# ZJU-DAILY/HC-SpMM

Hardware: AMD Instinct MI355X
Metric: GNN-aggregation SpMM edges*dim/s (A*X, fp32) (higher is better)
Workload: dtype f32

## Files before the change

hc-spmm_amd/csrc/capi.hip:

```cpp
#include <hip/hip_runtime.h>
#include <stdint.h>
#include <stdlib.h>

#include "fingerprint.h"
#include "graph_build.h"
#include "hcspmm.h"
#include "spmm_kernels.h"

namespace {
thread_local int g_last_hip_error = 0;

int fail_hip(hipError_t e) {
  g_last_hip_error = (int)e;
  return HCSPMM_EHIP;
}

inline bool aligned(const void* p, size_t a) { return (reinterpret_cast<uintptr_t>(p) & (a - 1)) == 0; }

constexpr int kDtypeF8 = HCSPMM_DTYPE_BF16 + 1;

inline int elem_bytes(int dtype) { return dtype == HCSPMM_DTYPE_F32 ? 4 : dtype == kDtypeF8 ? 1 : 2; }

int pick_vec(int dtype, int D, int64_t ldx, int64_t ldz, const void* X, const void* Z, const void* ws) {
  if (dtype == HCSPMM_DTYPE_F32) return D >= 4 ? 4 : D >= 2 ? 2 : 1;
// ... 233 lines not shown
  p.off_sched = ph->off_tasks;
  p.n_tasks = ph->n_tasks;
  p.n_tiny = ph->n_tiny;
  p.off_slice_table = ph->off_slice_table;
  p.off_slice_tasks = ph->off_slice_tasks;
  p.n_slices = ph->n_slices;
  p.slice_xcd_tasks = ph->slice_xcd_tasks;
  p.off_dense_index = ph->off_dense_index;
  p.off_dense_pack = ph->off_dense_pack;
  p.n_dense = ph->n_dense;
  p.off_dense_compact = ph->off_dense_compact;
  p.n_dense_compact = ph->n_dense_compact;
  p.off_dense_compact2 = ph->off_dense_compact2;
  p.n_dense_compact2 = ph->n_dense_compact2;
  p.off_fixups = ph->off_fixups;
  p.n_split_rows = ph->n_split_rows;
  wide_choice(ph, D, dtype, &p.n_wide, &p.panel_cols);
  return HCSPMM_OK;
}

inline void use_schedule(hcspmm::PlanArgs& p, const hcspmm_plan_header* ph) {
  if (ph->off_task_sched != 0) p.off_sched = ph->off_task_sched;
  if (ph->off_slice_sched != 0) p.off_slice_tasks = ph->off_slice_sched;
}

inline void set_operands(hcspmm::PlanArgs& p, const void* X, void* Z, int64_t ldx, int64_t ldz) {
  p.X = X;
  p.Z = Z;
  p.ldx = (size_t)ldx;
  p.ldz = (size_t)ldz;
}

inline hcspmm::WindowArgs window_args(const GraphIn& g, const hcspmm::PlanArgs& p) {
  return hcspmm::WindowArgs{p.X, p.Z, g.rowptr, g.col, g.blockPartition, g.edgeToColumn, g.edgeToRow, g.hybrid_type, p.ldx, p.ldz,
                            p.N, p.D};
}

template <class A>
using Launcher = hipError_t (*)(const A&, int, hipStream_t);
template <class A>
hipError_t launch_typed(int dtype, Launcher<A> f32, Launcher<A> f16, Launcher<A> bf16, const A& a, int vec, hipStream_t stream) {
  return (dtype == HCSPMM_DTYPE_F32 ? f32 : dtype == HCSPMM_DTYPE_F16 ? f16 : bf16)(a, vec, stream);
}

int forward_impl(const void* X, int64_t x_rows, int64_t ldx, void* Z, int64_t ldz, int dtype, const GraphIn& g, int D,
                 void* workspace, size_t workspace_bytes, void* stream_v, const FusedOperands* fused, const float* values = nullptr,
// ... 670 lines not shown
```

hc-spmm_amd/csrc/plan_host.cpp:

```cpp
#include <algorithm>
#include <atomic>
#include <chrono>
#include <condition_variable>
#include <cstdint>
#include <cstdio>
#include <cstdlib>
#include <cstring>
#include <mutex>
#include <thread>
#include <vector>

#include "fingerprint.h"
#include "hcspmm.h"
#include "host_util.h"

namespace {

constexpr int kSliceAuto = 0, kSliceOn = 1, kSliceOff = -1;
constexpr int32_t kSliceAutoThreshold = 256;
constexpr int64_t kSliceAutoMinColumns = 65536;
constexpr int64_t kSliceAutoAlwaysColumns = 250000;
constexpr int64_t kSliceAutoMinEntries = 3000000;
constexpr int kSliceSample = 4;
constexpr int64_t kScheduleMaxColumns = (256ll << 20) / 128;
constexpr int kSlicePad = 64;

struct Resolved {
  int32_t split_threshold, segment_len, fuse_in_launch;
  int32_t slice_mode, slice_threshold, n_slices, panel_cols;
  int32_t schedule;
};

int env_int(const char* name, int dflt) {
  const char* e = std::getenv(name);
  return e && *e ? std::atoi(e) : dflt;
}

Resolved resolve(const hcspmm_plan_params* p) {
  Resolved r{512, 256, 0, kSliceAuto, kSliceAutoThreshold, 8, 0, -1};
  if (p) {
    if (p->split_threshold > 0) r.split_threshold = p->split_threshold;
    if (p->segment_len > 0) r.segment_len = p->segment_len;
    r.fuse_in_launch = p->fuse_in_launch < 0 ? -1 : (p->fuse_in_launch > 2 ? 2 : p->fuse_in_launch);
  }
  if (r.segment_len > r.split_threshold) r.segment_len = r.split_threshold;
  int thr = p ? p->slice_threshold : 0, ns = p ? p->n_slices : 0;
  if (thr == 0) thr = env_int("HCSPMM_SLICE_THRESHOLD", 0);
  if (ns == 0) ns = env_int("HCSPMM_SLICES", 0);
  if (thr > 0) { r.slice_mode = kSliceOn; r.slice_threshold = thr; }
  else if (thr < 0) r.slice_mode = kSliceOff;
  if (ns > 0) r.n_slices = std::min(64, (ns + 7) / 8 * 8);
  r.schedule = env_int("HCSPMM_TASK_SCHEDULE", -1);
  if (p && p->panel_cols != 0) r.panel_cols = p->panel_cols < 0 ? -1 : std::min(1 << 20, (p->panel_cols + 15) / 16 * 16);
  return r;
}

inline int64_t pieces_bound(int64_t d, const Resolved& rp) {
  return std::min<int64_t>(d, rp.n_slices - 1 + (d + rp.segment_len - 1) / rp.segment_len);
}

inline void slice_cuts(const int32_t* col, int32_t e0, int64_t d, const int32_t* bounds, int S, int32_t* cuts) {
  const int32_t* first = col + e0;
  int64_t lo = 0;
  cuts[0] = 0;
  for (int s = 0; s < S; ++s) {
    const int64_t hi = (s == S - 1) ? d : std::lower_bound(first + lo, first + d, bounds[s]) - first;
    cuts[s + 1] = (int32_t)hi;
    lo = hi;
  }
}

template <typename F>
inline void for_each_piece(const int32_t* cuts, int32_t e0, int S, int32_t seg, F fn) {
  for (int s = 0; s < S; ++s)
    for (int64_t b = cuts[s]; b < cuts[s + 1]; b += seg) fn(s, (int32_t)(e0 + b), (int32_t)std::min<int64_t>(seg, cuts[s + 1] - b));
}

inline int64_t align4(int64_t x) { return (x + 3) & ~int64_t(3); }

struct Layout {
  int64_t n_tasks = 0, n_tiny = 0, n_dense = 0, n_compact = 0, n_compact2 = 0, n_split_rows = 0, n_partials = 0;
  int64_t dense_pack_words = 0;
  int64_t nnz_sparse = 0, nnz_dense = 0, dense_k_sum = 0;
  int32_t max_dense_k = 0;
  int64_t n_sparse_windows = 0;
  int64_t n_slice_tasks = 0, n_sliced_rows = 0, nnz_sliced = 0;
  int64_t off_tasks = 0, off_dense_index = 0, off_dense_pack = 0, off_compact2 = 0, off_compact = 0, off_fixups = 0,
          off_sparse_windows = 0, off_slice_table = 0, off_slice_tasks = 0, off_task_sched = 0, off_slice_sched = 0, total = 0;
};

class PassPool {
 public:
  explicit PassPool(int T) : T_(T) {
    for (int t = 1; t < T_; ++t) th_.emplace_back([this, t] { work(t); });
  }
  ~PassPool() {
    fn_ = nullptr;
    post();
    for (auto& x : th_) x.join();
  }
  int size() const { return T_; }
  template <typename F> void run(F& fn) {
    fn_ = [](void* f, int t) { (*static_cast<F*>(f))(t); };
    arg_ = &fn;
    done_.store(0, std::memory_order_relaxed);
    post();
    fn(0);
    for (int spin = 0; done_.load(std::memory_order_acquire) != T_ - 1; ++spin)
      if (spin > 256) std::this_thread::yield();
  }

// ... 104 lines not shown
    L.nnz_sparse += p.nnz_sparse; L.nnz_dense += p.nnz_dense; L.dense_k_sum += p.dense_k_sum;
    L.n_sparse_windows += p.n_sparse_windows;
    L.n_slice_tasks += p.n_slice_tasks; L.n_sliced_rows += p.n_sliced_rows; L.nnz_sliced += p.nnz_sliced;
    L.max_dense_k = std::max(L.max_dense_k, p.max_dense_k);
  }
  if (slicing) L.n_slice_tasks += (int64_t)kSlicePad * rp.n_slices;
  L.off_tasks = HCSPMM_PLAN_HEADER_WORDS;
  L.off_dense_index = align4(L.off_tasks + 4 * L.n_tasks);
  L.off_dense_pack = align4(L.off_dense_index + 4 * L.n_dense);
  L.off_compact2 = (L.off_dense_pack + L.dense_pack_words + 63) & ~int64_t(63);
  L.off_compact = L.off_compact2 + HCSPMM_COMPACT2_WORDS * L.n_compact2;
  L.off_fixups = align4(L.off_compact + HCSPMM_COMPACT_WORDS * L.n_compact);
  L.off_sparse_windows = align4(L.off_fixups + 4 * L.n_split_rows);
  L.off_slice_table = align4(L.off_sparse_windows + L.n_sparse_windows);
  L.off_slice_tasks = slicing ? align4(L.off_slice_table + rp.n_slices + 1) : L.off_slice_table;
  L.total = align4(L.off_slice_tasks + 4 * (slicing ? L.n_slice_tasks : 0));
  if (rp.schedule) {
    L.off_task_sched = L.total;
    L.total += 4 * (L.n_tasks - L.n_tiny);
    if (slicing) {
      L.off_slice_sched = L.total;
      L.total += 4 * L.n_slice_tasks;
    }
  }
  if (L.total > INT32_MAX) return HCSPMM_ERANGE;
  *out = L;
  return HCSPMM_OK;
}

void sort_by_length(const int32_t* src, int32_t* dst, int64_t n, int32_t max_len, int T) {
  if (n <= 0) return;
  if (n < 65536) T = 1;
  int32_t longest = 0;
  {
    std::vector<int32_t> part((size_t)T, 0);
    parallel_for(T, [&](int t) {
      int32_t m = 0;
      for (int64_t i = n * t / T; i < n * (t + 1) / T; ++i) m = std::max(m, src[4 * i + 2]);
      part[(size_t)t] = m;
    });
    for (int t = 0; t < T; ++t) longest = std::max(longest, part[(size_t)t]);
  }
  longest = std::min(longest, max_len);
  const size_t nb = (size_t)longest + 1;
  if (nb * (size_t)T > ((size_t)1 << 24)) T = 1;
  std::vector<std::vector<int64_t>> at((size_t)T);
  parallel_for(T, [&](int t) {
    std::vector<int64_t> h(nb, 0);
    for (int64_t i = n * t / T; i < n * (t + 1) / T; ++i) h[(size_t)std::min(std::max(src[4 * i + 2], 0), longest)]++;
    at[(size_t)t].swap(h);
// ... 75 lines not shown
}

extern "C" int hcspmm_plan_build(const int32_t* rowptr, const int32_t* col, int64_t N, int64_t E, int64_t M,
                                 const int32_t* bp, const int32_t* e2c, const int32_t* ht,
                                 const hcspmm_plan_params* params, int32_t* plan, int64_t words) {
  if (!rowptr || !plan || N < 0 || E < 0) return HCSPMM_EINVAL;
  if (N > 0 && (!bp || !ht)) return HCSPMM_EINVAL;
  if (E > 0 && (!col || !e2c)) return HCSPMM_EINVAL;
  if (N > INT32_MAX - 16 || E > INT32_MAX) return HCSPMM_ERANGE;
  if (M <= 0) M = N;
  if (M > INT32_MAX) return HCSPMM_ERANGE;
  PoolScope scope(plan_threads((N + HCSPMM_BLK_H - 1) / HCSPMM_BLK_H));
  static const bool dbg = std::getenv("HCSPMM_PLAN_DEBUG") != nullptr;
  auto now = [] { return std::chrono::duration<double, std::milli>(std::chrono::steady_clock::now().time_since_epoch()).count(); };
  double tp[8] = {now(), 0, 0, 0, 0, 0, 0, 0};
  uint64_t fingerprint = 0;
  {
    const int frc = fingerprint_and_check(rowptr, col, N, E, M, &fingerprint);
    if (frc != HCSPMM_OK) return frc;
  }
  tp[1] = now();
  Resolved rp = resolve(params);
  rp.schedule = rp.schedule < 0 ? (M <= kScheduleMaxColumns) : (rp.schedule != 0);
  Layout L;
  int rc = HCSPMM_OK;
  bool slicing = rp.slice_mode == kSliceOn;
  if (rp.slice_mode != kSliceOff) {
    rc = compute_layout(rowptr, N, bp, ht, rp, true, &L);
    if (rc != HCSPMM_OK) return rc;
    if (rp.slice_mode == kSliceAuto)
      slicing = M >= kSliceAutoMinColumns && L.nnz_sliced * 20 >= L.nnz_sparse && L.nnz_sliced > 0 &&
                (M >= kSliceAutoAlwaysColumns || L.nnz_sparse >= kSliceAutoMinEntries);
    if (L.n_sliced_rows == 0) slicing = false;
  }
  if (!slicing) {
    rc = compute_layout(rowptr, N, bp, ht, rp, false, &L);
    if (rc != HCSPMM_OK) return rc;
  }
  if (words < L.total) return HCSPMM_EINVAL;
  const int64_t W = (N + HCSPMM_BLK_H - 1) / HCSPMM_BLK_H;
  const int S = slicing ? rp.n_slices : 0;
  tp[2] = now();

  const int T = plan_threads(W);
  std::vector<int64_t> cut((size_t)T + 1);
  for (int t = 0; t <= T; ++t) cut[(size_t)t] = W * t / T;
// ... 204 lines not shown
         [&](int sl, int32_t row, int32_t first, int32_t len, int32_t slot_id) {
           const int64_t q = sp[(size_t)sl * (size_t)n_cls + (size_t)length_class(len)]++;
           sout[4 * q + 0] = row;
           sout[4 * q + 1] = first;
           sout[4 * q + 2] = len;
           sout[4 * q + 3] = slot_id;
         });
  });

  if (rp.schedule) {
    const int64_t n_nt = L.n_tasks - L.n_tiny;
    sort_by_length(out, plan + L.off_task_sched, n_nt, rp.split_threshold, T);
    if (slicing) {
      int32_t* ssched = plan + L.off_slice_sched;
      std::atomic<int> next_list{0};
      parallel_for(T, [&](int) {
        for (int sl; (sl = next_list.fetch_add(1, std::memory_order_relaxed)) < S;) {
          const int64_t lo = table[(size_t)sl], real = slice_real[(size_t)sl];
          sort_by_length(sout + 4 * lo, ssched + 4 * lo, real, rp.split_threshold, 1);
          std::memcpy(ssched + 4 * (lo + real), sout + 4 * (lo + real), 16 * (size_t)(table[(size_t)sl + 1] - lo - real));
        }
      });
      std::memset(ssched + 4 * table[(size_t)S], 0, 16 * (size_t)(L.n_slice_tasks - table[(size_t)S]));
    }
  }

  tp[5] = now();
  std::stable_sort(dense.begin(), dense.end(), [](const DenseRef& a, const DenseRef& b) { return a.K > b.K; });
  int32_t* dindex = plan + L.off_dense_index;
  int32_t* dpack = plan + L.off_dense_pack;
  const int64_t n_reg = L.n_dense - L.n_compact - L.n_compact2, n_c2 = L.n_compact2;
  std::vector<int64_t> pack_at((size_t)n_reg + 1, 0);
  for (int64_t i = 0; i < n_reg; ++i) pack_at[(size_t)i + 1] = pack_at[(size_t)i] + dense[(size_t)i].K + (dense[(size_t)i].K / 4) * 2;
  std::vector<int64_t> uniq_part((size_t)T, 0);
  std::vector<int> bad((size_t)T, 0);
  parallel_for(T, [&](int t) {
    int64_t uniq_total = 0;
    for (int64_t i = L.n_dense * t / T; i < L.n_dense * (t + 1) / T; ++i) {
      const int64_t w = dense[(size_t)i].w;
      const int32_t K = dense[(size_t)i].K, K4 = K / 4;
      const int64_t r0 = w * HCSPMM_BLK_H, r1 = std::min<int64_t>(r0 + HCSPMM_BLK_H, N);
      const int kind = i < n_reg ? 0 : (i < n_reg + n_c2 ? 2 : 1);
      if (kind != (K <= HCSPMM_COMPACT_K ? 1 : (K <= HCSPMM_COMPACT2_K ? 2 : 0))) { bad[(size_t)t] = 1; return; }
      const int32_t kmax = kind == 1 ? HCSPMM_COMPACT_K : (kind == 2 ? HCSPMM_COMPACT2_K : K);
      const int64_t off = kind == 1 ? HCSPMM_COMPACT_WORDS * (i - n_reg - n_c2)
                                    : (kind == 2 ? HCSPMM_COMPACT2_WORDS * (i - n_reg) : pack_at[(size_t)i]);
// ... 54 lines not shown
  h.n_tiny = (int32_t)n_tiny;
  h.n_dense_compact = (int32_t)L.n_compact;
  h.off_dense_compact = (int32_t)L.off_compact;
  h.n_dense_compact2 = (int32_t)L.n_compact2;
  h.off_dense_compact2 = (int32_t)L.off_compact2;
  h.num_columns = (int32_t)M;
  h.n_sparse_windows = (int32_t)L.n_sparse_windows;
  h.off_sparse_windows = (int32_t)L.off_sparse_windows;
  h.fingerprint_lo = (uint32_t)(fingerprint & 0xffffffffull);
  h.fingerprint_hi = (uint32_t)(fingerprint >> 32);
  h.dense_k_sum = (int32_t)std::min<int64_t>(L.dense_k_sum, INT32_MAX);
  h.flags = rp.fuse_in_launch < 0 ? HCSPMM_PLAN_FUSE_NEVER : (rp.fuse_in_launch >= 2 ? HCSPMM_PLAN_FUSE_ROWS : (rp.fuse_in_launch == 1 ? HCSPMM_PLAN_FUSE_IN_LAUNCH : 0));
  h.n_slices = S;
  h.slice_threshold = slicing ? rp.slice_threshold : 0;
  h.off_slice_table = (int32_t)L.off_slice_table;
  h.off_slice_tasks = (int32_t)L.off_slice_tasks;
  h.n_slice_tasks = slicing ? (int32_t)table[(size_t)S] : 0;
  h.slice_xcd_tasks = (int32_t)slice_xcd_tasks;
  h.nnz_sliced = slicing ? (int32_t)L.nnz_sliced : 0;
  h.n_sliced_rows = slicing ? (int32_t)L.n_sliced_rows : 0;
  h.panel_cols = rp.panel_cols;
  h.off_task_sched = (int32_t)L.off_task_sched;
  h.off_slice_sched = (int32_t)L.off_slice_sched;
  static_assert(sizeof(hcspmm_plan_header) == HCSPMM_PLAN_HEADER_WORDS * 4, "header size");
  std::memcpy(plan, &h, sizeof(h));
  if (dbg) {
    tp[6] = now();
    std::fprintf(stderr, "plan_build: T=%d: fingerprint + range check %.2f | layout %.2f | clear + slice boundaries %.2f | task pass 1 (count) %.2f | "
                         "task pass 2 (write) %.2f | dense packs %.2f | total %.2f ms\n",
                 T, tp[1] - tp[0], tp[2] - tp[1], tp[3] - tp[2], tp[4] - tp[3], tp[5] - tp[4], tp[6] - tp[5], tp[6] - tp[0]);
  }
  return HCSPMM_OK;
}

extern "C" int hcspmm_plan_check(const hcspmm_plan_header* h, int64_t N, int64_t E, int64_t words_available) {
  if (!h) return HCSPMM_EINVAL;
  if (h->magic != HCSPMM_PLAN_MAGIC || h->version != HCSPMM_PLAN_VERSION) return HCSPMM_EPLAN;
  if (h->num_nodes != N || h->num_edges != E) return HCSPMM_EPLAN;
  if (h->num_windows != (N + HCSPMM_BLK_H - 1) / HCSPMM_BLK_H) return HCSPMM_EPLAN;
  if (h->num_columns < 0 || (h->num_columns == 0 && N > 0)) return HCSPMM_EPLAN;
  if (h->n_tasks < 0 || h->n_dense < 0 || h->n_split_rows < 0 || h->n_partials < 0) return HCSPMM_EPLAN;
  if (h->n_tiny < 0 || h->n_tiny > h->n_tasks) return HCSPMM_EPLAN;
  if (h->n_dense_compact < 0 || h->n_dense_compact2 < 0 ||
      (int64_t)h->n_dense_compact + h->n_dense_compact2 > h->n_dense)
    return HCSPMM_EPLAN;
  if (h->n_sparse_windows < 0 || (int64_t)h->n_sparse_windows + h->n_dense != h->num_windows) return HCSPMM_EPLAN;
// ... 13 lines not shown
  if (h->off_sparse_windows < h->off_fixups + 4 * (int64_t)h->n_split_rows || (h->off_sparse_windows & 3)) return HCSPMM_EPLAN;
  if (h->total_words < h->off_sparse_windows + (int64_t)h->n_sparse_windows) return HCSPMM_EPLAN;
  if (h->n_slices < 0 || h->n_slices > 64 || (h->n_slices & 7) || h->n_slice_tasks < 0 || h->slice_xcd_tasks < 0) return HCSPMM_EPLAN;
  if (h->n_slices > 0) {
    if (h->slice_threshold <= 0 || (h->n_slice_tasks % 64) || (h->slice_xcd_tasks % 64) || h->slice_xcd_tasks > h->n_slice_tasks)
      return HCSPMM_EPLAN;
    if (h->off_slice_table < h->off_sparse_windows + (int64_t)h->n_sparse_windows || (h->off_slice_table & 3)) return HCSPMM_EPLAN;
    if (h->off_slice_tasks < h->off_slice_table + (int64_t)h->n_slices + 1 || (h->off_slice_tasks & 3)) return HCSPMM_EPLAN;
    if (h->total_words < h->off_slice_tasks + 4 * (int64_t)h->n_slice_tasks) return HCSPMM_EPLAN;
    if (h->nnz_sliced < 0 || h->nnz_sliced > h->nnz_sparse) return HCSPMM_EPLAN;
  } else if (h->n_slice_tasks != 0 || h->slice_xcd_tasks != 0) {
    return HCSPMM_EPLAN;
  }
  const int64_t lists_end = h->n_slices > 0 ? h->off_slice_tasks + 4 * (int64_t)h->n_slice_tasks
                                            : h->off_sparse_windows + (int64_t)h->n_sparse_windows;
  const int64_t n_nt = (int64_t)h->n_tasks - h->n_tiny;
  if (h->off_task_sched != 0 &&
      (h->off_task_sched < lists_end || (h->off_task_sched & 3) || h->total_words < h->off_task_sched + 4 * n_nt))
    return HCSPMM_EPLAN;
  if (h->off_slice_sched != 0 &&
      (h->n_slices == 0 || h->off_task_sched == 0 || h->off_slice_sched < h->off_task_sched + 4 * n_nt || (h->off_slice_sched & 3) ||
       h->total_words < h->off_slice_sched + 4 * (int64_t)h->n_slice_tasks))
    return HCSPMM_EPLAN;
  if (words_available > 0 && h->total_words > words_available) return HCSPMM_EPLAN;
  if ((int64_t)h->nnz_sparse + h->nnz_dense != E) return HCSPMM_EPLAN;
  return HCSPMM_OK;
}

extern "C" size_t hcspmm_workspace_bytes(const hcspmm_plan_header* h, int D) {
  if (!h || D <= 0) return 0;
  return (size_t)h->n_partials * (size_t)D * sizeof(float);
}
```

hc-spmm_amd/csrc/spmm_impl.h:

```cpp
#pragma once
#include <hip/hip_runtime.h>
#include <stdint.h>
#include <stdlib.h>

#include "hcspmm.h"
#include "spmm_kernels.h"
#include "plan_layout.h"

namespace hcspmm {

struct F32 { typedef float T; typedef float Z; };
struct F16 { typedef unsigned short T; typedef unsigned short Z; };
struct BF16 { typedef unsigned short T; typedef unsigned short Z; };
struct F8 { typedef unsigned char T; typedef float Z; };

typedef float f32x4 __attribute__((ext_vector_type(4)));
typedef unsigned int u32x4 __attribute__((ext_vector_type(4)));
typedef unsigned int u32x2 __attribute__((ext_vector_type(2)));

template <int VEC> struct AccT { typedef float type __attribute__((ext_vector_type(VEC))); };
template <> struct AccT<1> { typedef float type; };
__device__ __forceinline__ float aget(const float& v, int) { return v; }
__device__ __forceinline__ void aset(float& v, int, float x) { v = x; }
template <typename V> __device__ __forceinline__ float aget(const V& v, int i) { return v[i]; }
// ... 164 lines not shown
}

#ifndef HCSPMM_INDEX_VEC
#define HCSPMM_INDEX_VEC 4
#endif
#ifndef HCSPMM_INDEX_VEC_MIN
#define HCSPMM_INDEX_VEC_MIN 32
#endif

template <int IV>
__device__ __forceinline__ const int* index_source(const int* __restrict__ col, int e, int left, int nE,
                                                   typename IntV<IV>::type& v) {
  if (left <= 0) return nullptr;
  if constexpr (IV == 1) return col + e;
  else {
    if (e <= nE - IV) return col + e;
#pragma unroll
    for (int k = 0; k < IV; ++k)
      if (k < left) v[k] = col[e + k];
    return nullptr;
  }
}

template <typename E, int L, int VEC, bool WIDE, int UMAX, int IV>
__device__ __forceinline__ void sparse_task_body(const typename E::T* __restrict__ X, typename E::Z* __restrict__ dstZ,
                                                 float* __restrict__ dstP, const int* __restrict__ col, int nE, int e0, int n,
                                                 int nmax, size_t ldx, int c0, int cend, int lane) {
  typedef Lane<E, VEC> Ln;
  typedef typename Ln::acc_t acc_t;
  constexpr int U = (L < UMAX) ? L : UMAX;
  typedef typename IntV<IV>::type idx_t;
  typedef typename MemI32<IV>::type idx_mem_t;
  constexpr int STRIDE = WIDE ? 64 : L * IV;
  static_assert(IV == 1 || U % IV == 0, "a batch must start on a lane's first index");
  const int s = lane & (L - 1);
  const int pos = WIDE ? lane : s * IV;
  const int gbase = lane & ~(L - 1);

  for (int pbase = c0; pbase < cend; pbase += L * VEC) {
    const bool cok = pbase + s * VEC < cend;
    const int c = cok ? lane_col<VEC>(pbase + s * VEC, cend) : 0;
    const int csafe = c;
    acc_t acc = azero<VEC>();
    idx_t next = idx_t(-1);
    if (const int* p0 = index_source<IV>(col, e0 + pos, n - pos, nE, next)) next = *reinterpret_cast<const idx_mem_t*>(p0);
    for (int base = 0; base < nmax; base += STRIDE) {
      idx_t myidx = next;
      if constexpr (IV > 1) {
#pragma unroll
        for (int k = 1; k < IV; ++k) myidx[k] = (base + pos + k < n) ? myidx[k] : -1;
      }
      next = idx_t(-1);
      const int cnt = min(WIDE ? L : STRIDE, nmax - base);
      const int* pf = index_source<IV>(col, e0 + base + STRIDE + pos, n - (base + STRIDE + pos), nE, next);
      for (int j = 0; j < cnt;) {
        const int left = cnt - j;
        const int src = gbase + j / IV;
        if (left > U / 2) {
          gather_batch<E, VEC, U, IV>(X, ldx, csafe, cok, myidx, src, acc, pf, next);
          j += U;
        } else if (U >= 8 && left > U / 4) {
          gather_batch<E, VEC, (U >= 8 ? U / 2 : 1), IV>(X, ldx, csafe, cok, myidx, src, acc, pf, next);
          j += U / 2;
        } else if (U >= 4 && left > 1) {
          gather_batch<E, VEC, (U >= 8 ? U / 4 : 2), IV>(X, ldx, csafe, cok, myidx, src, acc, pf, next);
          j += (U >= 8 ? U / 4 : 2);
        } else {
          gather_batch<E, VEC, 1, IV>(X, ldx, csafe, cok, myidx, src, acc, pf, next);
          j += 1;
        }
        pf = nullptr;
      }
    }
    if (WIDE) {
#pragma unroll
      for (int off = L; off < 64; off <<= 1) {
#pragma unroll
        for (int q = 0; q < VEC; ++q) aset(acc, q, aget(acc, q) + __shfl_xor(aget(acc, q), off, 64));
      }
    }
    if (cok && (!WIDE || lane < L)) {
      if (dstZ != nullptr) Ln::store(dstZ + c, acc);
      else if (dstP != nullptr) Ln::store_partial(dstP + c, acc);
    }
  }
}

template <typename E, int L, int VEC, bool WIDE, int UMAX = HCSPMM_SPARSE_U, int IVREQ = 1>
__device__ __forceinline__ void sparse_task(const typename E::T* __restrict__ X, typename E::Z* __restrict__ dstZ,
                                            float* __restrict__ dstP, const int* __restrict__ col, int nE, int e0, int n,
                                            size_t ldx, int c0, int cend, int lane) {
  int nmax = n;
  if (!WIDE) {
#pragma unroll
    for (int off = L; off < 64; off <<= 1) nmax = max(nmax, __shfl_xor(nmax, off, 64));
  }
  nmax = __builtin_amdgcn_readfirstlane(nmax);
  constexpr int IV = (!WIDE && L == 8 && sizeof(typename E::T) == 4) ? IVREQ : 1;
  if constexpr (IV > 1) {
    if (nmax > HCSPMM_INDEX_VEC_MIN) {
      sparse_task_body<E, L, VEC, WIDE, UMAX, IV>(X, dstZ, dstP, col, nE, e0, n, nmax, ldx, c0, cend, lane);
      return;
    }
  }
  sparse_task_body<E, L, VEC, WIDE, UMAX, 1>(X, dstZ, dstP, col, nE, e0, n, nmax, ldx, c0, cend, lane);
}

template <typename E, int L, int VEC, int T>
__device__ __forceinline__ void tiny_tasks(const PlanArgs& a, int first, int c0, int cend, int lane) {
  typedef Lane<E, VEC> Ln;
  typedef typename E::T elem_t;
  const elem_t* X = reinterpret_cast<const elem_t*>(a.X);
  typename E::Z* Z = reinterpret_cast<typename E::Z*>(a.Z);
  constexpr int R = 64 / L;
  const int g = lane / L, s = lane & (L - 1);
  const int4* tasks = reinterpret_cast<const int4*>(a.plan + a.off_tasks);
  int4 d[T];
  bool any1 = false, any2 = false;
#pragma unroll
  for (int t = 0; t < T; ++t) {
    const int tid = first + t * R + g;
    d[t] = (tid < a.n_tasks) ? tasks[tid] : int4{0, -1, -1, -1};
  }
#pragma unroll
  for (int t = 0; t < T; ++t) {
    any1 |= d[t].y >= 0;
    any2 |= d[t].w >= 0;
  }
// ... 323 lines not shown
    const int p = (int)blockIdx.x / a.sparse_wgs_pp;
    const int b = (int)blockIdx.x - p * a.sparse_wgs_pp;
    const int c0 = p * a.panel_cols;
    const int cend = min(a.D, c0 + a.panel_cols);
    const int bf = b - a.slice_wgs;
    if (bf >= 0 && bf < a.wide_wgs) {
      const int tid = bf * kWaves + wave;
      if (tid >= a.n_wide) return;
      const int4 t = reinterpret_cast<const int4*>(a.plan + a.off_sched)[tid];
      typename E::Z* dz = (t.w < 0) ? Z + (size_t)t.x * a.ldz : nullptr;
      float* dp = (t.w < 0) ? nullptr : a.partial + (size_t)t.w * (size_t)a.D;
      sparse_task<E, L, VEC, true, UNROLL>(X, dz, dp, a.col, a.E, __builtin_amdgcn_readfirstlane(t.y),
                                           __builtin_amdgcn_readfirstlane(t.z), a.ldx, c0, cend, lane);
    } else if (bf >= sparse_wgs_pp_ordinary_end(a)) {
      if (bf >= a.free_wgs_pp) return;
      constexpr int R = 64 / L;
      const int first = a.n_tasks - a.n_tiny + ((bf - sparse_wgs_pp_ordinary_end(a)) * kWaves + wave) * (R * TinyT<L>::value);
      if (first >= a.n_tasks) return;
      tiny_tasks<E, L, VEC, TinyT<L>::value>(a, first, c0, cend, lane);
    } else {
      constexpr int R = 64 / L;
      const int g = lane / L;
      const int4* tp = nullptr;
      if (bf < 0) {
        cint_p tbl = (cint_p)(a.plan + a.off_slice_table);
        int j = ((b >> 3) * kWaves + wave) * R;
        for (int sl = b & 7; sl < a.n_slices; sl += 8) {
          const int lo = tbl[sl], cnt = tbl[sl + 1] - lo;
          if (j < cnt) {
            tp = reinterpret_cast<const int4*>(a.plan + a.off_slice_tasks) + lo + j + g;
            break;
          }
          j -= cnt;
        }
      } else {
        const int tid = a.n_wide + ((bf - a.wide_wgs) * kWaves + wave) * R + g;
        if (tid < a.n_tasks - a.n_tiny) tp = reinterpret_cast<const int4*>(a.plan + a.off_sched) + tid;
      }
      int e0 = 0, n = 0;
      typename E::Z* dz = nullptr;
      float* dp = nullptr;
      if (tp != nullptr) {
        const int4 t = *tp;
        if (t.x >= 0) {
          e0 = t.y;
          n = t.z;
          if (t.w < 0) dz = Z + (size_t)t.x * a.ldz;
          else dp = a.partial + (size_t)t.w * (size_t)a.D;
        }
      }
      sparse_task<E, L, VEC, false, UNROLL, HCSPMM_INDEX_VEC>(X, dz, dp, a.col, a.E, e0, n, a.ldx, c0, cend, lane);
    }
  } else {
    if constexpr (FUSED) {
      fused_dense_region(a, lane, wave);
      return;
    }
    constexpr int VM = DenseV<VEC>::mid;
    int unit = ((int)blockIdx.x - a.sparse_wgs) * kWaves + wave;
    if (unit >= a.n_dense * a.n_panels) return;
    const int n_reg = a.n_dense - a.n_dense_compact - a.n_dense_compact2;
    if (unit >= n_reg * a.n_panels) {
      unit -= n_reg * a.n_panels;
      if (unit < a.n_dense_compact2 * a.n_panels) {
        const int panel = unit / a.n_dense_compact2, ci = unit - panel * a.n_dense_compact2;
        const int* rec = a.plan + a.off_dense_compact2 + ci * HCSPMM_COMPACT2_WORDS;
        if (a.dense_vec == VEC) dense_compact_unit<E, VEC, 2>(X, Z, rec, panel, a.N, a.D, a.ldx, a.ldz, lane);
        else if (a.dense_vec == VM) dense_compact_unit<E, VM, 2>(X, Z, rec, panel, a.N, a.D, a.ldx, a.ldz, lane);
        else dense_compact_unit<E, 1, 2>(X, Z, rec, panel, a.N, a.D, a.ldx, a.ldz, lane);
        return;
      }
      unit -= a.n_dense_compact2 * a.n_panels;
      const int panel = unit / a.n_dense_compact, ci = unit - panel * a.n_dense_compact;
      const int* rec = a.plan + a.off_dense_compact + ci * HCSPMM_COMPACT_WORDS;
// ... 261 lines not shown
```

hc-spmm_amd/csrc/spmm_kernels.h:

```cpp
#pragma once
#include <hip/hip_runtime.h>
#include <stdint.h>

namespace hcspmm {

struct PlanArgs {
  const void* X;
  void* Z;
  float* partial;
  const int* col;
  const int* plan;
  size_t ldx, ldz;
  int off_tasks, n_tasks;
  int off_dense_index, off_dense_pack, n_dense;
  int off_dense_compact, n_dense_compact;
  int off_dense_compact2, n_dense_compact2;
  int off_fixups, n_split_rows;
  int N, D;
  int n_wide;
  int n_tiny;
  int panel_cols;
  int sparse_wgs_pp, dense_vec;
  int wide_wgs, sparse_wgs, n_panels;
  int tiny_wgs;
  int tiny_kernel_wgs;
  int off_slice_table, off_slice_tasks, n_slices, slice_xcd_tasks;
  int slice_wgs;
  int free_wgs_pp;
  int fused, H;
  int fused_dense_wgs;
  union {
    const float* W;
    const float* row_scale;
  };
  long long w_ldr, w_ldc;
  float* out;
  int E;
  int off_sched;
};

struct TilesArgs {
  PlanArgs p;
  int n_ord_tiles, n_tiny_tiles;
  int chunk, tile_stride;
};

struct WindowArgs {
  const void* X;
  void* Z;
  const int* rowptr;
  const int* col;
  const int* blockPartition;
  const int* edgeToColumn;
  const int* edgeToRow;
  const int* hybrid_type;
  size_t ldx, ldz;
  int N, D;
};

struct WPlanArgs {
  PlanArgs p;
// ... 200 lines not shown
```

hc-spmm_amd/hcspmm/capi.py:

```python
import ctypes
import os

_HERE = os.path.dirname(os.path.abspath(__file__))
LIB_PATH = os.environ.get("HCSPMM_LIB") or os.path.normpath(os.path.join(_HERE, "..", "csrc", "libhcspmm.so"))

RULE_INTENDED = 0
RULE_INTENDED_GUARD = 1
RULE_AS_SHIPPED = 2
RULE_MI355X = 3
RULE_MI355X_WIDE = 4

OK, EINVAL, ENOMEM, EPLAN, EHIP, EWORKSPACE, ERANGE = 0, -1, -2, -3, -4, -5, -6


class Header(ctypes.Structure):
    WORDS = 64
    MAGIC = 0x48435350
    _fields_ = [(n, ctypes.c_int32) for n in (
        "magic", "version", "total_words", "num_nodes", "num_edges", "num_windows", "split_threshold", "segment_len",
        "n_tasks", "n_dense", "n_split_rows", "n_partials", "off_tasks", "off_dense_index", "off_dense_pack",
        "off_fixups", "nnz_sparse", "nnz_dense", "uniq_dense", "max_dense_k")] + [("n_len_gt", ctypes.c_int32 * 5),
                                                                                  ("n_tiny", ctypes.c_int32), ("n_dense_compact", ctypes.c_int32),
                                                                                  ("off_dense_compact", ctypes.c_int32), ("n_dense_compact2", ctypes.c_int32),
                                                                                  ("off_dense_compact2", ctypes.c_int32), ("num_columns", ctypes.c_int32),
                                                                                  ("n_sparse_windows", ctypes.c_int32), ("off_sparse_windows", ctypes.c_int32),
                                                                                  ("fingerprint_lo", ctypes.c_uint32), ("fingerprint_hi", ctypes.c_uint32),
                                                                                  ("dense_k_sum", ctypes.c_int32), ("flags", ctypes.c_int32),
                                                                                  ("n_slices", ctypes.c_int32), ("slice_threshold", ctypes.c_int32),
                                                                                  ("off_slice_table", ctypes.c_int32), ("off_slice_tasks", ctypes.c_int32),
                                                                                  ("n_slice_tasks", ctypes.c_int32), ("slice_xcd_tasks", ctypes.c_int32),
                                                                                  ("nnz_sliced", ctypes.c_int32), ("n_sliced_rows", ctypes.c_int32),
                                                                                  ("panel_cols", ctypes.c_int32),
                                                                                  ("off_task_sched", ctypes.c_int32), ("off_slice_sched", ctypes.c_int32),
                                                                                  ("reserved", ctypes.c_int32 * 16)]

    @property
    def fingerprint(self):
        return (int(self.fingerprint_hi) << 32) | int(self.fingerprint_lo)


class PlanParams(ctypes.Structure):
    _fields_ = [("split_threshold", ctypes.c_int32), ("segment_len", ctypes.c_int32), ("fuse_in_launch", ctypes.c_int32),
                ("slice_threshold", ctypes.c_int32), ("n_slices", ctypes.c_int32), ("panel_cols", ctypes.c_int32)]


_vp, _i64, _int, _sz = ctypes.c_void_p, ctypes.c_int64, ctypes.c_int, ctypes.c_size_t
_hp, _pp = ctypes.POINTER(Header), ctypes.POINTER(PlanParams)
SYMBOLS = {
    "hcspmm_strerror": (ctypes.c_char_p, [_int]),
    "hcspmm_abi_version": (_int, []),
    "hcspmm_last_hip_error": (_int, []),
    "hcspmm_preprocess_host": (_int, [_vp, _vp, _i64, _i64, _i64, _int, _int, _vp, _vp, _vp, _vp]),
    "hcspmm_edge_to_row_device": (_int, [_vp, _i64, _i64, _vp, _vp]),
    "hcspmm_plan_words": (_int, [_vp, _i64, _i64, _vp, _vp, _pp, ctypes.POINTER(_i64)]),
    "hcspmm_plan_build": (_int, [_vp, _vp, _i64, _i64, _i64, _vp, _vp, _vp, _pp, _vp, _i64]),
    "hcspmm_plan_check": (_int, [_hp, _i64, _i64, _i64]),
    "hcspmm_graph_fingerprint_host": (_int, [_vp, _vp, _i64, _i64, ctypes.POINTER(ctypes.c_uint64)]),
    "hcspmm_graph_fingerprint_device": (_int, [_vp, _vp, _i64, _i64, _vp, _vp]),
    "hcspmm_workspace_bytes": (_sz, [_hp, _int]),
    "hcspmm_wide_threshold": (ctypes.c_int32, [_hp, _int]),
    "hcspmm_wide_threshold_typed": (ctypes.c_int32, [_hp, _int, _int]),
# ... 94 lines not shown
```

hc-spmm_amd/hybrid_kernel/hybrid_all.cpp:

```cpp
#include <torch/extension.h>

#include <c10/hip/HIPStream.h>

#include <cstring>
#include <mutex>
#include <string>
#include <tuple>
#include <unordered_map>
#include <vector>

#include "hcspmm.h"

namespace {

#define CHECK_CUDA(x) TORCH_CHECK(x.is_cuda(), #x " must be a CUDA tensor")
#define CHECK_CONTIGUOUS(x) TORCH_CHECK(x.is_contiguous(), #x " must be contiguous")
#define CHECK_INPUT(x) \
  CHECK_CUDA(x);       \
  CHECK_CONTIGUOUS(x)

int g_rule = HCSPMM_RULE_MI355X;
hcspmm_plan_params g_params = {0, 0, 0, 0, 0, 0};

void check_rc(int rc, const char* what) {
// ... 1417 lines not shown
    if (need == 0) return torch::Tensor();
    auto ws = torch::empty({(int64_t)(need / 4)}, A.options());
    auto out = torch::empty({(int64_t)D, (int64_t)H}, A.options());
    const c10::DeviceGuard guard(A.device());
    check_rc(hcspmm_weight_grad(A.data_ptr<float>(), A.stride(0), B.data_ptr<float>(), B.stride(0), out.data_ptr<float>(), N,
                                D, H, ws.data_ptr(), need, current_stream(A)),
             "weight_grad");
    return out;
  }, "dW = A^T B for the layers' backward passes (split-K MFMA kernel); None if the shape is unsupported");
  m.def("plan_info", [](torch::Tensor row_nzr) {
    pybind11::dict d;
    hcspmm_plan_header h;
    if (!read_plan_header(row_nzr, &h)) return d;
    d["n_tasks"] = h.n_tasks; d["n_dense"] = h.n_dense; d["n_split_rows"] = h.n_split_rows;
    d["n_partials"] = h.n_partials; d["nnz_sparse"] = h.nnz_sparse; d["nnz_dense"] = h.nnz_dense;
    d["uniq_dense"] = h.uniq_dense; d["split_threshold"] = h.split_threshold; d["segment_len"] = h.segment_len;
    d["max_dense_k"] = h.max_dense_k; d["n_tiny"] = h.n_tiny; d["n_dense_compact"] = h.n_dense_compact;
    d["n_dense_compact2"] = h.n_dense_compact2; d["num_columns"] = h.num_columns;
    d["panel_cols"] = h.panel_cols; d["n_slices"] = h.n_slices; d["slice_threshold"] = h.slice_threshold; d["n_slice_tasks"] = h.n_slice_tasks;
    d["nnz_sliced"] = h.nnz_sliced; d["n_sliced_rows"] = h.n_sliced_rows; d["total_words"] = h.total_words;
    d["n_sparse_windows"] = h.n_sparse_windows; d["dense_k_sum"] = h.dense_k_sum; d["flags"] = h.flags; d["num_nodes"] = h.num_nodes; d["num_edges"] = h.num_edges;
    d["fingerprint"] = ((uint64_t)h.fingerprint_hi << 32) | h.fingerprint_lo;
    d["off_task_sched"] = h.off_task_sched; d["off_slice_sched"] = h.off_slice_sched;
    return d;
  }, "fields of the launch plan carried in row_nzr ({} for the reference's [0] placeholder)");
}
```

include/hcspmm.h:

```cpp
#ifndef HCSPMM_H
#define HCSPMM_H

#include <stddef.h>
#include <stdint.h>

#ifdef __cplusplus
extern "C" {
#endif

#define HCSPMM_ABI_VERSION 3

#define HCSPMM_BLK_H 16
#define HCSPMM_BLK_W 8

#define HCSPMM_OK 0
#define HCSPMM_EINVAL (-1)
#define HCSPMM_ENOMEM (-2)
#define HCSPMM_EPLAN (-3)
#define HCSPMM_EHIP (-4)
#define HCSPMM_EWORKSPACE (-5)
#define HCSPMM_ERANGE (-6)

#define HCSPMM_RULE_INTENDED 0
#define HCSPMM_RULE_INTENDED_GUARD 1
// ... 1 lines not shown
#define HCSPMM_RULE_MI355X 3
#define HCSPMM_RULE_MI355X_WIDE 4

const char* hcspmm_strerror(int code);
int hcspmm_abi_version(void);
int hcspmm_last_hip_error(void);

int hcspmm_preprocess_host(const int32_t* row_pointers_h, const int32_t* column_index_h, int64_t num_nodes,
                           int64_t num_edges, int64_t num_columns, int rule, int num_threads,
                           int32_t* blockPartition_h, int32_t* edgeToColumn_h, int32_t* edgeToRow_h,
                           int32_t* hybrid_type_h);

int hcspmm_edge_to_row_device(const int32_t* row_pointers_d, int64_t num_nodes, int64_t num_edges, int32_t* edgeToRow_d,
                              void* stream);

#define HCSPMM_PLAN_MAGIC 0x48435350
#define HCSPMM_PLAN_VERSION 8
#define HCSPMM_TINY_LEN 2
#define HCSPMM_COMPACT_K 40
#define HCSPMM_COMPACT_WORDS 64
#define HCSPMM_COMPACT2_K 80
#define HCSPMM_COMPACT2_WORDS 128
#define HCSPMM_PLAN_HEADER_WORDS 64

typedef struct hcspmm_plan_header {
  int32_t magic;
  int32_t version;
  int32_t total_words;
  int32_t num_nodes;
  int32_t num_edges;
  int32_t num_windows;
  int32_t split_threshold;
  int32_t segment_len;
  int32_t n_tasks;
  int32_t n_dense;
  int32_t n_split_rows;
  int32_t n_partials;
  int32_t off_tasks;
  int32_t off_dense_index;
  int32_t off_dense_pack;
  int32_t off_fixups;
  int32_t nnz_sparse;
  int32_t nnz_dense;
  int32_t uniq_dense;
  int32_t max_dense_k;
  int32_t n_len_gt[5];
  int32_t n_tiny;
  int32_t n_dense_compact;
  int32_t off_dense_compact;
  int32_t n_dense_compact2;
  int32_t off_dense_compact2;
  int32_t num_columns;
  int32_t n_sparse_windows;
  int32_t off_sparse_windows;
  uint32_t fingerprint_lo;
  uint32_t fingerprint_hi;
  int32_t dense_k_sum;
  int32_t flags;
  int32_t n_slices;
  int32_t slice_threshold;
  int32_t off_slice_table;
  int32_t off_slice_tasks;
  int32_t n_slice_tasks;
  int32_t slice_xcd_tasks;
  int32_t nnz_sliced;
  int32_t n_sliced_rows;
  int32_t panel_cols;
  int32_t off_task_sched;
  int32_t off_slice_sched;
  int32_t reserved[16];
} hcspmm_plan_header;

#define HCSPMM_PLAN_FUSE_IN_LAUNCH 1
#define HCSPMM_PLAN_FUSE_ROWS 2
#define HCSPMM_PLAN_FUSE_NEVER 4

typedef struct hcspmm_plan_params {
  int32_t split_threshold;
  int32_t segment_len;
  int32_t fuse_in_launch;
  int32_t slice_threshold;
  int32_t n_slices;
  int32_t panel_cols;
} hcspmm_plan_params;

int hcspmm_plan_words(const int32_t* row_pointers_h, int64_t num_nodes, int64_t num_edges,
                      const int32_t* blockPartition_h, const int32_t* hybrid_type_h,
                      const hcspmm_plan_params* params, int64_t* words_out);

int hcspmm_plan_build(const int32_t* row_pointers_h, const int32_t* column_index_h, int64_t num_nodes,
                      int64_t num_edges, int64_t num_columns, const int32_t* blockPartition_h,
                      const int32_t* edgeToColumn_h, const int32_t* hybrid_type_h, const hcspmm_plan_params* params,
                      int32_t* plan_h, int64_t words);
// ... 262 lines not shown
```

Measured before the change: 4016 billion.

## Embed first column-index chunk per scheduled task in plan records

```diff
diff --git a/hc-spmm_amd/csrc/capi.hip b/hc-spmm_amd/csrc/capi.hip
--- a/hc-spmm_amd/csrc/capi.hip
+++ b/hc-spmm_amd/csrc/capi.hip
@@ -279,6 +279,14 @@
 inline void use_schedule(hcspmm::PlanArgs& p, const hcspmm_plan_header* ph) {
   if (ph->off_task_sched != 0) p.off_sched = ph->off_task_sched;
   if (ph->off_slice_sched != 0) p.off_slice_tasks = ph->off_slice_sched;
+  if (ph->off_task_sched != 0 && ph->off_task_sched_idx != 0) p.off_sched_idx = ph->off_task_sched_idx;
+  if (ph->off_slice_sched != 0 && ph->off_slice_sched_idx != 0) {
+    p.off_slice_idx = ph->off_slice_sched_idx;
+    if (ph->n_slices == 8) {
+      p.slice_tbl_n = 9;
+      for (int s = 0; s < 9; ++s) p.slice_tbl[s] = ph->slice_table_copy[s];
+    }
+  }
 }
 
 inline void set_operands(hcspmm::PlanArgs& p, const void* X, void* Z, int64_t ldx, int64_t ldz) {
diff --git a/hc-spmm_amd/csrc/plan_host.cpp b/hc-spmm_amd/csrc/plan_host.cpp
--- a/hc-spmm_amd/csrc/plan_host.cpp
+++ b/hc-spmm_amd/csrc/plan_host.cpp
@@ -23,12 +23,14 @@
 constexpr int64_t kSliceAutoMinEntries = 3000000;
 constexpr int kSliceSample = 4;
 constexpr int64_t kScheduleMaxColumns = (256ll << 20) / 128;
+constexpr int64_t kIdxWords = HCSPMM_SCHED_INDEX_WORDS;
 constexpr int kSlicePad = 64;
 
 struct Resolved {
   int32_t split_threshold, segment_len, fuse_in_launch;
   int32_t slice_mode, slice_threshold, n_slices, panel_cols;
   int32_t schedule;
+  int32_t sched_index;
 };
 
 int env_int(const char* name, int dflt) {
@@ -37,7 +39,7 @@
 }
 
 Resolved resolve(const hcspmm_plan_params* p) {
-  Resolved r{512, 256, 0, kSliceAuto, kSliceAutoThreshold, 8, 0, -1};
+  Resolved r{512, 256, 0, kSliceAuto, kSliceAutoThreshold, 8, 0, -1, 1};
   if (p) {
     if (p->split_threshold > 0) r.split_threshold = p->split_threshold;
     if (p->segment_len > 0) r.segment_len = p->segment_len;
@@ -51,6 +53,7 @@
   else if (thr < 0) r.slice_mode = kSliceOff;
   if (ns > 0) r.n_slices = std::min(64, (ns + 7) / 8 * 8);
   r.schedule = env_int("HCSPMM_TASK_SCHEDULE", -1);
+  r.sched_index = env_int("HCSPMM_SCHED_INDEX", 1) != 0;
   if (p && p->panel_cols != 0) r.panel_cols = p->panel_cols < 0 ? -1 : std::min(1 << 20, (p->panel_cols + 15) / 16 * 16);
   return r;
 }
@@ -86,7 +89,7 @@
   int64_t n_sparse_windows = 0;
   int64_t n_slice_tasks = 0, n_sliced_rows = 0, nnz_sliced = 0;
   int64_t off_tasks = 0, off_dense_index = 0, off_dense_pack = 0, off_compact2 = 0, off_compact = 0, off_fixups = 0,
-          off_sparse_windows = 0, off_slice_table = 0, off_slice_tasks = 0, off_task_sched = 0, off_slice_sched = 0, total = 0;
+          off_sparse_windows = 0, off_slice_table = 0, off_slice_tasks = 0, off_task_sched = 0, off_slice_sched = 0, off_task_sched_idx = 0, off_slice_sched_idx = 0, total = 0;
 };
 
 class PassPool {
@@ -237,10 +240,31 @@
       L.off_slice_sched = L.total;
       L.total += 4 * L.n_slice_tasks;
     }
+    if (rp.sched_index) {
+      L.off_task_sched_idx = (L.total + kIdxWords - 1) / kIdxWords * kIdxWords;
+      L.total = L.off_task_sched_idx + kIdxWords * (L.n_tasks - L.n_tiny);
+      if (slicing) {
+        L.off_slice_sched_idx = L.total;
+        L.total += kIdxWords * L.n_slice_tasks;
+      }
+    }
   }
   if (L.total > INT32_MAX) return HCSPMM_ERANGE;
   *out = L;
   return HCSPMM_OK;
+}
+
+void first_index_records(const int32_t* desc, int32_t* rec, int64_t n, int64_t n_all, const int32_t* col, int T) {
+  if (n_all < 4096) T = 1;
+  parallel_for(T, [&](int t) {
+    for (int64_t i = n_all * t / T; i < n_all * (t + 1) / T; ++i) {
+      int32_t* r = rec + kIdxWords * i;
+      const int32_t* d = desc + 4 * i;
+      const int64_t k = (i < n && d[0] >= 0) ? std::min<int64_t>(std::max(d[2], 0), kIdxWords) : 0;
+      if (k > 0) std::memcpy(r, col + d[1], sizeof(int32_t) * (size_t)k);
+      for (int64_t j = k; j < kIdxWords; ++j) r[j] = -1;
+    }
+  });
 }
 
 void sort_by_length(const int32_t* src, int32_t* dst, int64_t n, int32_t max_len, int T) {
@@ -362,6 +386,7 @@
   tp[1] = now();
   Resolved rp = resolve(params);
   rp.schedule = rp.schedule < 0 ? (M <= kScheduleMaxColumns) : (rp.schedule != 0);
+  rp.sched_index = rp.schedule && rp.sched_index;
   Layout L;
   int rc = HCSPMM_OK;
   bool slicing = rp.slice_mode == kSliceOn;
@@ -612,6 +637,12 @@
         }
       });
       std::memset(ssched + 4 * table[(size_t)S], 0, 16 * (size_t)(L.n_slice_tasks - table[(size_t)S]));
+    }
+    if (L.off_task_sched_idx) {
+      std::memset(plan + L.off_task_sched + 4 * n_nt + (slicing ? 4 * L.n_slice_tasks : 0), 0,
+                  sizeof(int32_t) * (size_t)(L.off_task_sched_idx - (L.off_task_sched + 4 * n_nt + (slicing ? 4 * L.n_slice_tasks : 0))));
+      first_index_records(plan + L.off_task_sched, plan + L.off_task_sched_idx, n_nt, n_nt, col, T);
+      if (slicing) first_index_records(plan + L.off_slice_sched, plan + L.off_slice_sched_idx, table[(size_t)S], L.n_slice_tasks, col, T);
     }
   }
 
@@ -712,6 +743,10 @@
   h.panel_cols = rp.panel_cols;
   h.off_task_sched = (int32_t)L.off_task_sched;
   h.off_slice_sched = (int32_t)L.off_slice_sched;
+  h.off_task_sched_idx = (int32_t)L.off_task_sched_idx;
+  h.off_slice_sched_idx = (int32_t)L.off_slice_sched_idx;
+  if (L.off_slice_sched_idx && S == 8)
+    for (int s = 0; s <= S; ++s) h.slice_table_copy[s] = (int32_t)table[(size_t)s];
   static_assert(sizeof(hcspmm_plan_header) == HCSPMM_PLAN_HEADER_WORDS * 4, "header size");
   std::memcpy(plan, &h, sizeof(h));
   if (dbg) {
@@ -771,6 +806,23 @@
       (h->n_slices == 0 || h->off_task_sched == 0 || h->off_slice_sched < h->off_task_sched + 4 * n_nt || (h->off_slice_sched & 3) ||
        h->total_words < h->off_slice_sched + 4 * (int64_t)h->n_slice_tasks))
     return HCSPMM_EPLAN;
+  const int64_t sched_end = h->off_slice_sched != 0 ? h->off_slice_sched + 4 * (int64_t)h->n_slice_tasks : h->off_task_sched + 4 * n_nt;
+  if (h->off_task_sched_idx != 0 &&
+      (h->off_task_sched == 0 || h->off_task_sched_idx < sched_end || (h->off_task_sched_idx % kIdxWords) ||
+       h->total_words < h->off_task_sched_idx + kIdxWords * n_nt))
+    return HCSPMM_EPLAN;
+  if (h->off_slice_sched_idx != 0 &&
+      (h->off_slice_sched == 0 || h->off_task_sched_idx == 0 || h->off_slice_sched_idx < h->off_task_sched_idx + kIdxWords * n_nt ||
+       (h->off_slice_sched_idx % kIdxWords) || h->total_words < h->off_slice_sched_idx + kIdxWords * (int64_t)h->n_slice_tasks))
+    return HCSPMM_EPLAN;
+  if (h->off_slice_sched_idx != 0 && h->n_slices == 8) {
+    if (h->slice_table_copy[0] != 0 || h->slice_table_copy[8] != h->n_slice_tasks) return HCSPMM_EPLAN;
+    for (int s = 0; s < 8; ++s)
+      if (h->slice_table_copy[s + 1] < h->slice_table_copy[s] || (h->slice_table_copy[s] % 64)) return HCSPMM_EPLAN;
+  } else {
+    for (int s = 0; s < 9; ++s)
+      if (h->slice_table_copy[s] != 0) return HCSPMM_EPLAN;
+  }
   if (words_available > 0 && h->total_words > words_available) return HCSPMM_EPLAN;
   if ((int64_t)h->nnz_sparse + h->nnz_dense != E) return HCSPMM_EPLAN;
   return HCSPMM_OK;
diff --git a/hc-spmm_amd/csrc/spmm_impl.h b/hc-spmm_amd/csrc/spmm_impl.h
--- a/hc-spmm_amd/csrc/spmm_impl.h
+++ b/hc-spmm_amd/csrc/spmm_impl.h
@@ -210,10 +210,12 @@
   }
 }
 
-template <typename E, int L, int VEC, bool WIDE, int UMAX, int IV>
+template <typename E, int L, int VEC, bool WIDE, int UMAX, int IV, bool FC = false>
 __device__ __forceinline__ void sparse_task_body(const typename E::T* __restrict__ X, typename E::Z* __restrict__ dstZ,
                                                  float* __restrict__ dstP, const int* __restrict__ col, int nE, int e0, int n,
-                                                 int nmax, size_t ldx, int c0, int cend, int lane) {
+                                                 int nmax, size_t ldx, int c0, int cend, int lane, bool have_first = false,
+                                                 typename IntV<IV>::type first = typename IntV<IV>::type(-1),
+                                                 const int* __restrict__ rec = nullptr) {
   typedef Lane<E, VEC> Ln;
   typedef typename Ln::acc_t acc_t;
   constexpr int U = (L < UMAX) ? L : UMAX;
@@ -224,14 +226,28 @@
   const int s = lane & (L - 1);
   const int pos = WIDE ? lane : s * IV;
   const int gbase = lane & ~(L - 1);
-
+  auto chunk_source = [&](int at, idx_t& v) -> const int* {
+    if constexpr (FC && IV == 1 && !WIDE) {
+      static_assert(!FC || 32 % L == 0, "a chunk lies inside the record or behind it");
+      if (have_first && at < 32) return at + pos < n ? rec + at + pos : nullptr;
+    }
+    return index_source<IV>(col, e0 + at + pos, n - (at + pos), nE, v);
+  };
+
+  idx_t next = idx_t(-1);
+  if constexpr (FC) {
+    if (have_first) next = first;
+    else if (const int* p0 = chunk_source(0, next)) next = *reinterpret_cast<const idx_mem_t*>(p0);
+  }
   for (int pbase = c0; pbase < cend; pbase += L * VEC) {
     const bool cok = pbase + s * VEC < cend;
     const int c = cok ? lane_col<VEC>(pbase + s * VEC, cend) : 0;
     const int csafe = c;
     acc_t acc = azero<VEC>();
-    idx_t next = idx_t(-1);
-    if (const int* p0 = index_source<IV>(col, e0 + pos, n - pos, nE, next)) next = *reinterpret_cast<const idx_mem_t*>(p0);
+    if constexpr (!FC) {
+      next = idx_t(-1);
+      if (const int* p0 = index_source<IV>(col, e0 + pos, n - pos, nE, next)) next = *reinterpret_cast<const idx_mem_t*>(p0);
+    }
     for (int base = 0; base < nmax; base += STRIDE) {
       idx_t myidx = next;
       if constexpr (IV > 1) {
@@ -240,7 +256,7 @@
       }
       next = idx_t(-1);
       const int cnt = min(WIDE ? L : STRIDE, nmax - base);
-      const int* pf = index_source<IV>(col, e0 + base + STRIDE + pos, n - (base + STRIDE + pos), nE, next);
+      const int* pf = chunk_source(base + STRIDE, next);
       for (int j = 0; j < cnt;) {
         const int left = cnt - j;
         const int src = gbase + j / IV;
@@ -271,13 +287,21 @@
       if (dstZ != nullptr) Ln::store(dstZ + c, acc);
       else if (dstP != nullptr) Ln::store_partial(dstP + c, acc);
     }
-  }
-}
-
-template <typename E, int L, int VEC, bool WIDE, int UMAX = HCSPMM_SPARSE_U, int IVREQ = 1>
+    if constexpr (FC) {
+      if (pbase + L * VEC < cend) {
+        next = idx_t(-1);
+        if (const int* p0 = chunk_source(0, next)) next = *reinterpret_cast<const idx_mem_t*>(p0);
+      }
+    }
+  }
+}
+
+template <typename E, int L, int VEC, bool WIDE, int UMAX = HCSPMM_SPARSE_U, int IVREQ = 1, bool FC = false>
 __device__ __forceinline__ void sparse_task(const typename E::T* __restrict__ X, typename E::Z* __restrict__ dstZ,
                                             float* __restrict__ dstP, const int* __restrict__ col, int nE, int e0, int n,
-                                            size_t ldx, int c0, int cend, int lane) {
+                                            size_t ldx, int c0, int cend, int lane, bool have_first = false,
+                                            typename IntV<IVREQ>::type first4 = typename IntV<IVREQ>::type(-1), int first1 = -1,
+                                            const int* __restrict__ rec = nullptr) {
   int nmax = n;
   if (!WIDE) {
 #pragma unroll
@@ -286,12 +310,13 @@
   nmax = __builtin_amdgcn_readfirstlane(nmax);
   constexpr int IV = (!WIDE && L == 8 && sizeof(typename E::T) == 4) ? IVREQ : 1;
   if constexpr (IV > 1) {
-    if (nmax > HCSPMM_INDEX_VEC_MIN) {
-      sparse_task_body<E, L, VEC, WIDE, UMAX, IV>(X, dstZ, dstP, col, nE, e0, n, nmax, ldx, c0, cend, lane);
+    if (nmax > HCSPMM_INDEX_VEC_MIN || (FC && have_first)) {
+      sparse_task_body<E, L, VEC, WIDE, UMAX, IV, FC>(X, dstZ, dstP, col, nE, e0, n, nmax, ldx, c0, cend, lane, have_first, first4);
       return;
     }
   }
-  sparse_task_body<E, L, VEC, WIDE, UMAX, 1>(X, dstZ, dstP, col, nE, e0, n, nmax, ldx, c0, cend, lane);
+  sparse_task_body<E, L, VEC, WIDE, UMAX, 1, FC>(X, dstZ, dstP, col, nE, e0, n, nmax, ldx, c0, cend, lane, IV == 1 && have_first,
+                                                 first1, rec);
 }
 
 template <typename E, int L, int VEC, int T>
@@ -661,26 +686,54 @@
       constexpr int R = 64 / L;
       const int g = lane / L;
       const int4* tp = nullptr;
+      constexpr bool FC = !FUSED && L <= 32;
+      constexpr bool FC4 = FC && L == 8 && sizeof(elem_t) == 4 && HCSPMM_INDEX_VEC == 4;
+      const int* rec = nullptr;
+      bool have_first = false;
       if (bf < 0) {
-        cint_p tbl = (cint_p)(a.plan + a.off_slice_table);
         int j = ((b >> 3) * kWaves + wave) * R;
-        for (int sl = b & 7; sl < a.n_slices; sl += 8) {
-          const int lo = tbl[sl], cnt = tbl[sl + 1] - lo;
-          if (j < cnt) {
-            tp = reinterpret_cast<const int4*>(a.plan + a.off_slice_tasks) + lo + j + g;
-            break;
+        int at = -1;
+        if (FC && a.slice_tbl_n != 0) {
+          const int lo = a.slice_tbl[b & 7], cnt = a.slice_tbl[(b & 7) + 1] - lo;
+          if (j < cnt) at = lo + j;
+        } else {
+          cint_p tbl = (cint_p)(a.plan + a.off_slice_table);
+          for (int sl = b & 7; sl < a.n_slices; sl += 8) {
+            const int lo = tbl[sl], cnt = tbl[sl + 1] - lo;
+            if (j < cnt) {
+              at = lo + j;
+              break;
+            }
+            j -= cnt;
           }
-          j -= cnt;
-        }
+        }
+        if (at >= 0) {
+          tp = reinterpret_cast<const int4*>(a.plan + a.off_slice_tasks) + at + g;
+          if (FC && a.off_slice_idx != 0) rec = a.plan + a.off_slice_idx + (size_t)(at + g) * 32;
+        }
+        have_first = FC && a.off_slice_idx != 0;
       } else {
         const int tid = a.n_wide + ((bf - a.wide_wgs) * kWaves + wave) * R + g;
-        if (tid < a.n_tasks - a.n_tiny) tp = reinterpret_cast<const int4*>(a.plan + a.off_sched) + tid;
+        if (tid < a.n_tasks - a.n_tiny) {
+          tp = reinterpret_cast<const int4*>(a.plan + a.off_sched) + tid;
+          if (FC && a.off_sched_idx != 0) rec = a.plan + a.off_sched_idx + (size_t)tid * 32;
+        }
+        have_first = FC && a.off_sched_idx != 0;
       }
       int e0 = 0, n = 0;
       typename E::Z* dz = nullptr;
       float* dp = nullptr;
+      typename IntV<HCSPMM_INDEX_VEC>::type first4 = typename IntV<HCSPMM_INDEX_VEC>::type(-1);
+      int first1 = -1;
       if (tp != nullptr) {
         const int4 t = *tp;
+        if constexpr (FC) {
+          if (rec != nullptr) {
+            const int sl = lane & (L - 1);
+            if constexpr (FC4) first4 = *reinterpret_cast<const typename IntV<HCSPMM_INDEX_VEC>::type*>(rec + 4 * sl);
+            else first1 = rec[sl];
+          }
+        }
         if (t.x >= 0) {
           e0 = t.y;
           n = t.z;
@@ -688,7 +741,8 @@
           else dp = a.partial + (size_t)t.w * (size_t)a.D;
         }
       }
-      sparse_task<E, L, VEC, false, UNROLL, HCSPMM_INDEX_VEC>(X, dz, dp, a.col, a.E, e0, n, a.ldx, c0, cend, lane);
+      sparse_task<E, L, VEC, false, UNROLL, HCSPMM_INDEX_VEC, FC>(X, dz, dp, a.col, a.E, e0, n, a.ldx, c0, cend, lane, have_first,
+                                                                  first4, first1, rec);
     }
   } else {
     if constexpr (FUSED) {
diff --git a/hc-spmm_amd/csrc/spmm_kernels.h b/hc-spmm_amd/csrc/spmm_kernels.h
--- a/hc-spmm_amd/csrc/spmm_kernels.h
+++ b/hc-spmm_amd/csrc/spmm_kernels.h
@@ -37,6 +37,9 @@
   float* out;
   int E;
   int off_sched;
+  int off_sched_idx, off_slice_idx;
+  int slice_tbl_n;
+  int slice_tbl[9];
 };
 
 struct TilesArgs {
diff --git a/hc-spmm_amd/hcspmm/capi.py b/hc-spmm_amd/hcspmm/capi.py
--- a/hc-spmm_amd/hcspmm/capi.py
+++ b/hc-spmm_amd/hcspmm/capi.py
@@ -37,6 +37,26 @@
     @property
     def fingerprint(self):
         return (int(self.fingerprint_hi) << 32) | int(self.fingerprint_lo)
+
+    @property
+    def off_task_sched_idx(self):
+        return int(self.reserved[0])
+
+    @off_task_sched_idx.setter
+    def off_task_sched_idx(self, v):
+        self.reserved[0] = v
+
+    @property
+    def off_slice_sched_idx(self):
+        return int(self.reserved[1])
+
+    @off_slice_sched_idx.setter
+    def off_slice_sched_idx(self, v):
+        self.reserved[1] = v
+
+    @property
+    def slice_table_copy(self):
+        return [int(v) for v in self.reserved[2:11]]
 
 
 class PlanParams(ctypes.Structure):
diff --git a/hc-spmm_amd/hybrid_kernel/hybrid_all.cpp b/hc-spmm_amd/hybrid_kernel/hybrid_all.cpp
--- a/hc-spmm_amd/hybrid_kernel/hybrid_all.cpp
+++ b/hc-spmm_amd/hybrid_kernel/hybrid_all.cpp
@@ -1463,6 +1463,7 @@
     d["n_sparse_windows"] = h.n_sparse_windows; d["dense_k_sum"] = h.dense_k_sum; d["flags"] = h.flags; d["num_nodes"] = h.num_nodes; d["num_edges"] = h.num_edges;
     d["fingerprint"] = ((uint64_t)h.fingerprint_hi << 32) | h.fingerprint_lo;
     d["off_task_sched"] = h.off_task_sched; d["off_slice_sched"] = h.off_slice_sched;
+    d["off_task_sched_idx"] = h.off_task_sched_idx; d["off_slice_sched_idx"] = h.off_slice_sched_idx;
     return d;
   }, "fields of the launch plan carried in row_nzr ({} for the reference's [0] placeholder)");
 }
diff --git a/include/hcspmm.h b/include/hcspmm.h
--- a/include/hcspmm.h
+++ b/include/hcspmm.h
@@ -47,6 +47,7 @@
 #define HCSPMM_COMPACT2_K 80
 #define HCSPMM_COMPACT2_WORDS 128
 #define HCSPMM_PLAN_HEADER_WORDS 64
+#define HCSPMM_SCHED_INDEX_WORDS 32
 
 typedef struct hcspmm_plan_header {
   int32_t magic;
@@ -93,7 +94,10 @@
   int32_t panel_cols;
   int32_t off_task_sched;
   int32_t off_slice_sched;
-  int32_t reserved[16];
+  int32_t off_task_sched_idx;
+  int32_t off_slice_sched_idx;
+  int32_t slice_table_copy[9];
+  int32_t reserved[5];
 } hcspmm_plan_header;
 
 #define HCSPMM_PLAN_FUSE_IN_LAUNCH 1
```

New measurement: 4125 billion, median of 6. 1.03x the previous value.
